# SaeedRahmani/AV-Simulation-at-Intersections

Measured on NVIDIA B200. Metric: batched MPC step solves/sec, higher is better.
Workload: dtype f64

## Files before the change

### av-simulation-at-intersections_b200/csrc/jmpc.cu

```cuda
#include <cuda_runtime.h>

#include <cstdio>
#include <cstdlib>
#include <cstring>
#include <new>
#include <string>
#include <chrono>
#include <vector>

#include "../../include/jmpc.h"
#include "jmpc_collision.cuh"
#include "jmpc_step.cuh"
#include "jmpc_episode.cuh"
#include "jmpc_planner.cuh"
#include "jmpc_courses.cuh"

namespace {

thread_local std::string g_err;

int fail(const char* what, cudaError_t e = cudaSuccess) {
  char buf[512];
  if (e != cudaSuccess) snprintf(buf, sizeof buf, "%s: %s", what, cudaGetErrorString(e));
  else snprintf(buf, sizeof buf, "%s", what);
// ... 1486 lines not shown
      B, h->n_courses, h->course_stride, course_id, course_ok, dl, h->d_cx, h->d_cy, h->d_cyaw, state, params, done);
  CK(cudaGetLastError());
  h->launches++;
  return 0;
}

int64_t jmpc_launch_count(jmpc_handle h) { return h ? h->launches : 0; }

int32_t jmpc_debug_linalg(jmpc_handle h, int32_t n, const double* A, const double* b, const double* x, double* sol,
                          double* prod) {
  return jmpc_debug_linalg_g(h, n, 32, 0, A, b, x, sol, prod);
}

int32_t jmpc_debug_linalg_g(jmpc_handle h, int32_t n, int32_t group_lanes, int32_t which, const double* A,
                            const double* b, const double* x, double* sol, double* prod) {
  if (!h || !A || !b || !x || !sol || !prod) return fail("jmpc_debug_linalg: NULL argument");
  if (n < 1 || n > 2 * JMPC_MAX_T) return fail("jmpc_debug_linalg: n out of range");
  if (group_lanes != 16 && group_lanes != 32) return fail("jmpc_debug_linalg: group_lanes must be 16 or 32");
  const int groups = 32 / group_lanes;
  if (which < 0 || which >= groups) return fail("jmpc_debug_linalg: no such lane group");
  CK(cudaSetDevice(h->device));
  const size_t nn = (size_t)n * n;
  const size_t in_doubles = nn + 2 * (size_t)n, out_doubles = 4 * (size_t)n + 2;
  if (ensure_stage(h, (in_doubles + out_doubles) * sizeof(double))) return -1;
  double* hs = (double*)h->h_stage;
  double* d = (double*)h->d_stage;
  memcpy(hs, A, nn * sizeof(double)); memcpy(hs + nn, b, n * sizeof(double)); memcpy(hs + nn + n, x, n * sizeof(double));
  double *dA = d, *db = dA + nn, *dx = db + n, *dsol = dx + n, *dprod = dsol + 2 * n;
  int* dok = (int*)(dprod + 2 * n);
  cudaStream_t st = h->own_stream;
  CK(cudaMemcpyAsync(d, hs, in_doubles * sizeof(double), cudaMemcpyHostToDevice, st));
  CK(cudaMemsetAsync(dsol, 0xff, out_doubles * sizeof(double), st));
  const int nb = jmpc::nblk(n);
  const size_t smem = (size_t)groups * (jmpc::tiles_doubles(n) + 8 * nb) * sizeof(double) +
                      jmpc::chol_lut_bytes(nb) + 16;
  if (group_lanes == 32) jmpc::linalg_selftest_kernel<32><<<1, 32, smem, st>>>(n, which, dA, db, dx, dsol, dprod, dok);
  else jmpc::linalg_selftest_kernel<16><<<1, 32, smem, st>>>(n, which, dA, db, dx, dsol, dprod, dok);
  CK(cudaGetLastError());
  h->launches++;
  CK(cudaMemcpyAsync(hs + in_doubles, dsol, out_doubles * sizeof(double), cudaMemcpyDeviceToHost, st));
  CK(cudaStreamSynchronize(st));
  memcpy(sol, hs + in_doubles, 2 * (size_t)n * sizeof(double));
  memcpy(prod, hs + in_doubles + 2 * n, 2 * (size_t)n * sizeof(double));
  int ok = 0;
  memcpy(&ok, hs + in_doubles + 4 * n, sizeof(int));
  return ok == 1 ? 0 : 1;
}

int32_t jmpc_measure_fma_peak(jmpc_handle h, double* fp64_tflops, double* fp32_tflops) {
  if (!h || !fp64_tflops || !fp32_tflops) return fail("jmpc_measure_fma_peak: NULL argument");
  CK(cudaSetDevice(h->device));
  if (measure_fma<double>(h, fp64_tflops)) return -1;
  if (measure_fma<float>(h, fp32_tflops)) return -1;
  return 0;
}

}
```

### av-simulation-at-intersections_b200/csrc/jmpc_linalg.cuh

```cuda
#pragma once
#include <cuda_runtime.h>
#include <math.h>

namespace jmpc {

#ifdef JMPC_UNROLL_BLOCKS
#define JMPC_PRAGMA_CHOL _Pragma("unroll")
#define JMPC_PRAGMA_SWEEP _Pragma("unroll")
#define JMPC_PRAGMA_SYMV _Pragma("unroll")
#else
#define JMPC_PRAGMA_CHOL _Pragma("unroll 1")
#define JMPC_PRAGMA_SWEEP _Pragma("unroll 1")
#define JMPC_PRAGMA_SYMV _Pragma("unroll 1")
#endif

#ifdef JMPC_CYCLES
__device__ unsigned long long g_cycles[32];
#define JMPC_TICK(var) long long var = clock64()
#define JMPC_TOCK(var, slot) do { long long now_ = clock64(); if ((threadIdx.x & 31) == 0) atomicAdd(&g_cycles[slot], (unsigned long long)(now_ - var)); var = now_; } while (0)
#else
#define JMPC_TICK(var)
#define JMPC_TOCK(var, slot)
#endif

constexpr int kTS = 18;
constexpr unsigned kFullMask = 0xffffffffu;

__host__ __device__ inline int nblk(int n) { return (n + 3) >> 2; }
__host__ __device__ inline int tiles_doubles(int n) { const int nb = nblk(n); return (nb * (nb + 1) / 2) * kTS; }
__host__ __device__ __forceinline__ int tile_off(int I, int J) { return (((I * (I + 1)) >> 1) + J) * kTS; }
__host__ __device__ __forceinline__ int elem_off(int i, int j) { return tile_off(i >> 2, j >> 2) + ((i & 3) << 2) + (j & 3); }

__device__ __forceinline__ double rsqrt_pos(double a) {
  double y;
  asm("rsqrt.approx.ftz.f64 %0, %1;" : "=d"(y) : "d"(a));
  const double e = fma(-a, y * y, 1.0);
  return fma(fma(e, 0.375, 0.5), y * e, y);
}
__device__ __forceinline__ double rcp_pos(double a) {
  double y;
  asm("rcp.approx.ftz.f64 %0, %1;" : "=d"(y) : "d"(a));
  double e = fma(-a, y, 1.0);
  y = fma(y, e, y);
  e = fma(-a, y, 1.0);
  return fma(y, e, y);
}
__device__ __forceinline__ double pivot_rsqrt(double a, bool& clean) {
  const double y = rsqrt_pos(a);
  const bool pos = a > 0.0;
  clean = clean && pos;
  return pos ? y : 0.0;
}

__device__ __forceinline__ void ld4(const double* p, double& a, double& b, double& c, double& d) {
  const double2 x = *reinterpret_cast<const double2*>(p), y = *reinterpret_cast<const double2*>(p + 2);
  a = x.x; b = x.y; c = y.x; d = y.y;
}
__device__ __forceinline__ void st4(double* p, double a, double b, double c, double d) {
  *reinterpret_cast<double2*>(p) = make_double2(a, b);
  *reinterpret_cast<double2*>(p + 2) = make_double2(c, d);
}

typedef unsigned int chol_task;
__host__ __device__ inline int chol_lut_entries(int nb) { return ((nb - 1) * nb * (nb + 1)) / 3; }
__host__ __device__ __forceinline__ int chol_lut_offset(int m) { return ((m - 1) * m * (m + 1)) / 3; }
__host__ __device__ inline size_t chol_lut_bytes(int nb) { return ((size_t)chol_lut_entries(nb) * sizeof(chol_task) + 15) & ~(size_t)15; }
__device__ inline void chol_lut_build(chol_task* lut, int nb, int tid, int nthreads) {
  for (int m = 1; m < nb; ++m) {
    const int ntasks = m * (m + 1), off = chol_lut_offset(m);
    const int J = nb - 1 - m;
    for (int q = tid; q < ntasks; q += nthreads) {
      const int t = q >> 1;
      int a = (int)((sqrtf(8.0f * (float)t + 1.0f) - 1.0f) * 0.5f);
      while (((a + 1) * (a + 2) >> 1) <= t) ++a;
      while (((a * (a + 1)) >> 1) > t) --a;
      const int b = t - ((a * (a + 1)) >> 1);
      const int I = J + 1 + a, Kc = J + 1 + b;
      lut[off + q] = ((unsigned)(b + 1) << 16) | ((unsigned)(q & 1) << 22) | (unsigned)(((I * (I + 1)) >> 1) + J) |
                     ((unsigned)(((Kc * (Kc + 1)) >> 1) + J) << 8);
    }
  }
}

template <int G>
__device__ inline bool chol_tiles(double* K, int nb, int gl, unsigned gm, const chol_task* lut,
                                  double* rhs = nullptr) {
  bool all_clean = true;
  JMPC_PRAGMA_CHOL
  for (int J = 0; J < nb; ++J) {
    JMPC_TICK(tc_);
    const double* D = K + tile_off(J, J);
    double a00, a10, a11, a20, a21, a22, a30, a31, a32, a33;
    {
      double u01, u02, u03, u12, u13, u23;
      ld4(D, a00, u01, u02, u03); ld4(D + 4, a10, a11, u12, u13);
      ld4(D + 8, a20, a21, a22, u23); ld4(D + 12, a30, a31, a32, a33);
      (void)u01; (void)u02; (void)u03; (void)u12; (void)u13; (void)u23;
    }
    bool clean = true;
    const double r0 = pivot_rsqrt(a00, clean);
    const double l10 = a10 * r0, l20 = a20 * r0, l30 = a30 * r0;
    a11 = fma(-l10, l10, a11);
    const double r1 = pivot_rsqrt(a11, clean);
    const double l21 = fma(-l20, l10, a21) * r1, l31 = fma(-l30, l10, a31) * r1;
    a22 = fma(-l21, l21, fma(-l20, l20, a22));
    const double r2 = pivot_rsqrt(a22, clean);
    const double l32 = fma(-l31, l21, fma(-l30, l20, a32)) * r2;
    a33 = fma(-l32, l32, fma(-l31, l31, fma(-l30, l30, a33)));
    const double r3 = pivot_rsqrt(a33, clean);
    all_clean = all_clean && clean;
    const double m00 = r0, m11 = r1, m22 = r2, m33 = r3;
    const double m10 = -(l10 * m00) * r1;
    const double m21 = -(l21 * m11) * r2;
    const double m32 = -(l32 * m22) * r3;
    const double m20 = -fma(l21, m10, l20 * m00) * r2;
    const double m31 = -fma(l32, m21, l31 * m11) * r3;
    const double m30 = -fma(l32, m20, fma(l31, m10, l30 * m00)) * r3;
    double y0 = 0.0, y1 = 0.0, y2 = 0.0, y3 = 0.0;
    if (rhs) {
      double b0, b1, b2, b3;
      ld4(rhs + (J << 2), b0, b1, b2, b3);
      y0 = m00 * b0; y1 = fma(m11, b1, m10 * b0); y2 = fma(m22, b2, fma(m21, b1, m20 * b0));
      y3 = fma(m31, b1, m30 * b0) + fma(m33, b3, m32 * b2);
    }
    __syncwarp(gm);
    JMPC_TOCK(tc_, 13);
    const int prow = (nb - J - 1) << 2;
    for (int r = gl; r < prow; r += G) {
      double* row = K + tile_off(J + 1 + (r >> 2), J) + ((r & 3) << 2);
      double a0, a1, a2, a3;
      ld4(row, a0, a1, a2, a3);
      const double x0 = a0 * m00, x1 = fma(a1, m11, a0 * m10), x2 = fma(a2, m22, fma(a1, m21, a0 * m20));
      const double x3 = fma(a3, m33, fma(a2, m32, fma(a1, m31, a0 * m30)));
      st4(row, x0, x1, x2, x3);
      if (rhs) {
        double* bi = rhs + ((J + 1) << 2) + r;
        *bi -= fma(x1, y1, x0 * y0) + fma(x3, y3, x2 * y2);
      }
    }
    if (gl == 0) {
      double* Mw = K + tile_off(J, J);
      st4(Mw, m00, 0.0, 0.0, 0.0); st4(Mw + 4, m10, m11, 0.0, 0.0);
      st4(Mw + 8, m20, m21, m22, 0.0); st4(Mw + 12, m30, m31, m32, m33);
      if (rhs) st4(rhs + (J << 2), y0, y1, y2, y3);
    }
    __syncwarp(gm);
    JMPC_TOCK(tc_, 14);
    const int m = nb - J - 1, ntasks = m * (m + 1);
    const chol_task* tasks = lut + chol_lut_offset(m);
    for (int q = gl; q < ntasks; q += G) {
      const unsigned e = tasks[q];
      const unsigned sLI = e & 255u, sLK = (e >> 8) & 255u, sC = sLI + ((e >> 16) & 15u), hb = (e >> 16) & 0x40u;
      const char* Kh = reinterpret_cast<const char*>(K) + hb;
      const double* LI = reinterpret_cast<const double*>(Kh + sLI * (unsigned)(kTS * sizeof(double)));
      const double* LK = K + sLK * (unsigned)kTS;
      double* C = reinterpret_cast<double*>(const_cast<char*>(Kh) + sC * (unsigned)(kTS * sizeof(double)));
      double k00, k01, k02, k03, k10, k11, k12, k13, k20, k21, k22, k23, k30, k31, k32, k33;
      ld4(LK, k00, k01, k02, k03); ld4(LK + 4, k10, k11, k12, k13);
      ld4(LK + 8, k20, k21, k22, k23); ld4(LK + 12, k30, k31, k32, k33);
#pragma unroll
      for (int r = 0; r < 2; ++r) {
        double x0, x1, x2, x3, c0, c1, c2, c3;
        ld4(LI + 4 * r, x0, x1, x2, x3);
        ld4(C + 4 * r, c0, c1, c2, c3);
        c0 = fma(-x3, k03, fma(-x2, k02, fma(-x1, k01, fma(-x0, k00, c0))));
        c1 = fma(-x3, k13, fma(-x2, k12, fma(-x1, k11, fma(-x0, k10, c1))));
        c2 = fma(-x3, k23, fma(-x2, k22, fma(-x1, k21, fma(-x0, k20, c2))));
        c3 = fma(-x3, k33, fma(-x2, k32, fma(-x1, k31, fma(-x0, k30, c3))));
        st4(C + 4 * r, c0, c1, c2, c3);
      }
    }
    __syncwarp(gm);
    JMPC_TOCK(tc_, 15);
  }
  return all_clean;
}

template <int G>
__device__ inline void solve_forward_tiles(const double* K, double* b, int nb, int gl, unsigned gm) {
  const int n4 = nb << 2;
  JMPC_PRAGMA_SWEEP
  for (int J = 0; J < nb; ++J) {
    const double* Mw = K + tile_off(J, J);
    double b0, b1, b2, b3;
    ld4(b + (J << 2), b0, b1, b2, b3);
    const double m00 = Mw[0];
    const double2 mr1 = *reinterpret_cast<const double2*>(Mw + 4);
    const double m10 = mr1.x, m11 = mr1.y;
    double m20, m21, m22, mpad, m30, m31, m32, m33;
    ld4(Mw + 8, m20, m21, m22, mpad); ld4(Mw + 12, m30, m31, m32, m33);
    (void)mpad;
    const double y0 = m00 * b0, y1 = fma(m11, b1, m10 * b0), y2 = fma(m22, b2, fma(m21, b1, m20 * b0));
    const double y3 = fma(m33, b3, fma(m32, b2, fma(m31, b1, m30 * b0)));
    __syncwarp(gm);
    for (int i = ((J + 1) << 2) + gl; i < n4; i += G) {
      double l0, l1, l2, l3;
      ld4(K + tile_off(i >> 2, J) + ((i & 3) << 2), l0, l1, l2, l3);
      b[i] = fma(-l3, y3, fma(-l2, y2, fma(-l1, y1, fma(-l0, y0, b[i]))));
    }
    if (gl == 0) st4(b + (J << 2), y0, y1, y2, y3);
    __syncwarp(gm);
  }
}
template <int G>
__device__ inline void solve_backward_tiles(const double* K, double* b, int nb, int gl, unsigned gm) {
  JMPC_PRAGMA_SWEEP
  for (int J = nb - 1; J >= 0; --J) {
    const double* Mw = K + tile_off(J, J);
    double y0, y1, y2, y3;
    ld4(b + (J << 2), y0, y1, y2, y3);
    const double m00 = Mw[0];
    const double2 mr1 = *reinterpret_cast<const double2*>(Mw + 4);
    const double m10 = mr1.x, m11 = mr1.y;
    double m20, m21, m22, mpad, m30, m31, m32, m33;
    ld4(Mw + 8, m20, m21, m22, mpad); ld4(Mw + 12, m30, m31, m32, m33);
    (void)mpad;
    const double x3 = m33 * y3, x2 = fma(m32, y3, m22 * y2), x1 = fma(m31, y3, fma(m21, y2, m11 * y1));
    const double x0 = fma(m30, y3, fma(m20, y2, fma(m10, y1, m00 * y0)));
    __syncwarp(gm);
    for (int i = gl; i < (J << 2); i += G) {
      const double* col = K + tile_off(J, i >> 2) + (i & 3);
      b[i] = fma(-col[12], x3, fma(-col[8], x2, fma(-col[4], x1, fma(-col[0], x0, b[i]))));
    }
    if (gl == 0) st4(b + (J << 2), x0, x1, x2, x3);
    __syncwarp(gm);
  }
}

template <int G>
__device__ __forceinline__ void sweep_load(const double* b, int n4, int gl, double& lo, double& hi) {
  lo = (gl < n4) ? b[gl] : 0.0;
  hi = (gl + G < n4) ? b[gl + G] : 0.0;
}
template <int G>
__device__ __forceinline__ void sweep_store(double* b, int n4, int gl, double lo, double hi) {
  if (gl < n4) b[gl] = lo;
  if (gl + G < n4) b[gl + G] = hi;
}
struct DiagInv { double m00, m10, m11, m20, m21, m22, m30, m31, m32, m33; };
__device__ __forceinline__ DiagInv load_diag_inv(const double* Mw) {
  DiagInv d;
  d.m00 = Mw[0];
  const double2 r1 = *reinterpret_cast<const double2*>(Mw + 4);
  d.m10 = r1.x; d.m11 = r1.y;
  double pad;
  ld4(Mw + 8, d.m20, d.m21, d.m22, pad); ld4(Mw + 12, d.m30, d.m31, d.m32, d.m33);
  (void)pad;
  return d;
}
template <int G, bool HI>
__device__ __forceinline__ void forward_block(const double* K, int J, int n4, int gl, unsigned gm, const double* row_lo,
                                              const double* row_hi, double& lo, double& hi) {
  double& own = HI ? hi : lo;
  const int l0 = (J << 2) & (G - 1);
  const double* Mw = K + tile_off(J, J);
  const int first = (J + 1) << 2;
  const bool act_lo = !HI && gl >= first && gl < n4, act_hi = gl + G >= first && gl + G < n4;
  double a0 = 0.0, a1 = 0.0, a2 = 0.0, a3 = 0.0, c0, c1, c2, c3;
  if (!HI) ld4(act_lo ? row_lo + J * kTS : Mw, a0, a1, a2, a3);
  ld4(act_hi ? row_hi + J * kTS : Mw, c0, c1, c2, c3);
  const DiagInv d = load_diag_inv(Mw);
  const double e0 = __shfl_sync(gm, own, l0, G), e1 = __shfl_sync(gm, own, l0 + 1, G);
  const double e2 = __shfl_sync(gm, own, l0 + 2, G), e3 = __shfl_sync(gm, own, l0 + 3, G);
  const double y0 = d.m00 * e0, y1 = fma(d.m11, e1, d.m10 * e0), y2 = fma(d.m22, e2, fma(d.m21, e1, d.m20 * e0));
  const double y3 = fma(d.m33, e3, fma(d.m32, e2, fma(d.m31, e1, d.m30 * e0)));
  if (!HI) {
    const double v = fma(-a3, y3, fma(-a2, y2, fma(-a1, y1, fma(-a0, y0, lo))));
    lo = act_lo ? v : lo;
  }
  {
    const double v = fma(-c3, y3, fma(-c2, y2, fma(-c1, y1, fma(-c0, y0, hi))));
    hi = act_hi ? v : hi;
  }
  const double s01 = (gl & 1) ? y1 : y0, s23 = (gl & 1) ? y3 : y2, mine = (gl & 2) ? s23 : s01;
  own = ((gl >> 2) == (l0 >> 2)) ? mine : own;
}
template <int G>
__device__ __forceinline__ void solve_forward_regs(const double* K, int nb, int gl, unsigned gm, double& lo, double& hi) {
  const int n4 = nb << 2;
  const double* row_lo = K + tile_off(gl >> 2, 0) + ((gl & 3) << 2);
  const double* row_hi = K + tile_off((gl + G) >> 2, 0) + ((gl & 3) << 2);
  const int nlo = nb < G / 4 ? nb : G / 4;
#pragma unroll 1
  for (int J = 0; J < nlo; ++J) forward_block<G, false>(K, J, n4, gl, gm, row_lo, row_hi, lo, hi);
#pragma unroll 1
  for (int J = G / 4; J < nb; ++J) forward_block<G, true>(K, J, n4, gl, gm, row_lo, row_hi, lo, hi);
}
template <int G, bool HI>
__device__ __forceinline__ void backward_block(const double* K, int J, int n4, int gl, unsigned gm, int col_lo, int col_hi,
                                               double& lo, double& hi) {
  double& own = HI ? hi : lo;
  const int l0 = (J << 2) & (G - 1);
  const double* Krow = K + tile_off(J, 0);
  const double* Mw = Krow + J * kTS;
  const int below = J << 2;
  const bool act_lo = gl < below && gl < n4, act_hi = HI && gl + G < below;
  const double* pa = act_lo ? Krow + col_lo : Mw;
  const double a0 = pa[0], a1 = pa[4], a2 = pa[8], a3 = pa[12];
  double c0 = 0.0, c1 = 0.0, c2 = 0.0, c3 = 0.0;
  if (HI) { const double* pc = act_hi ? Krow + col_hi : Mw; c0 = pc[0]; c1 = pc[4]; c2 = pc[8]; c3 = pc[12]; }
  const DiagInv d = load_diag_inv(Mw);
  const double y0 = __shfl_sync(gm, own, l0, G), y1 = __shfl_sync(gm, own, l0 + 1, G);
  const double y2 = __shfl_sync(gm, own, l0 + 2, G), y3 = __shfl_sync(gm, own, l0 + 3, G);
  const double x3 = d.m33 * y3, x2 = fma(d.m32, y3, d.m22 * y2), x1 = fma(d.m31, y3, fma(d.m21, y2, d.m11 * y1));
  const double x0 = fma(d.m30, y3, fma(d.m20, y2, fma(d.m10, y1, d.m00 * y0)));
  {
    const double v = fma(-a3, x3, fma(-a2, x2, fma(-a1, x1, fma(-a0, x0, lo))));
    lo = act_lo ? v : lo;
  }
  if (HI) {
    const double v = fma(-c3, x3, fma(-c2, x2, fma(-c1, x1, fma(-c0, x0, hi))));
    hi = act_hi ? v : hi;
  }
  const double s01 = (gl & 1) ? x1 : x0, s23 = (gl & 1) ? x3 : x2, mine = (gl & 2) ? s23 : s01;
  own = ((gl >> 2) == (l0 >> 2)) ? mine : own;
}
template <int G>
__device__ __forceinline__ void solve_backward_regs(const double* K, int nb, int gl, unsigned gm, double& lo, double& hi) {
  const int n4 = nb << 2;
  const int col_lo = (gl >> 2) * kTS + (gl & 3), col_hi = ((gl + G) >> 2) * kTS + (gl & 3);
#pragma unroll 1
  for (int J = nb - 1; J >= G / 4; --J) backward_block<G, true>(K, J, n4, gl, gm, col_lo, col_hi, lo, hi);
  const int nlo = nb < G / 4 ? nb : G / 4;
#pragma unroll 1
  for (int J = nlo - 1; J >= 0; --J) backward_block<G, false>(K, J, n4, gl, gm, col_lo, col_hi, lo, hi);
}

__device__ inline void symv_tiles(const double* P, const double* x, int nb, int lane,
                                  double& y0, double& y1) {
  const int n4 = nb << 2;
  y0 = 0.0; y1 = 0.0;
#pragma unroll
  for (int pass = 0; pass < 2; ++pass) {
    const int i = lane + 32 * pass;
    if (i < n4) {
      const int I = i >> 2, r = i & 3;
      double acc0 = 0.0, acc1 = 0.0;
      for (int J = 0; J <= I; ++J) {
        double p0, p1, p2, p3, x0, x1, x2, x3;
        ld4(P + tile_off(I, J) + (r << 2), p0, p1, p2, p3);
        ld4(x + (J << 2), x0, x1, x2, x3);
        acc0 = fma(p1, x1, fma(p0, x0, acc0));
        acc1 = fma(p3, x3, fma(p2, x2, acc1));
      }
      for (int J = I + 1; J < nb; ++J) {
        const double* col = P + tile_off(J, I) + r;
        double x0, x1, x2, x3;
        ld4(x + (J << 2), x0, x1, x2, x3);
        acc0 = fma(col[4], x1, fma(col[0], x0, acc0));
        acc1 = fma(col[12], x3, fma(col[8], x2, acc1));
      }
      if (pass == 0) y0 = acc0 + acc1; else y1 = acc0 + acc1;
    }
  }
}


template <int G>
__device__ inline void solve_tiles(const double* K, double* b, int nb, int gl, unsigned gm) {
  solve_forward_tiles<G>(K, b, nb, gl, gm);
  solve_backward_tiles<G>(K, b, nb, gl, gm);
}

template <int NB>
__device__ __forceinline__ void symv_rows(const double* P, const double* x, int T, int nb_rt, int gl, double& y0,
                                          double& y1) {
  const int nb = (NB > 0) ? NB : nb_rt;
  const bool own = gl < T;
  const int ia = own ? gl : 0, ib = own ? T + gl : 0;
  const int Ia = ia >> 2, Ib = ib >> 2;
  const double* rowa = P + tile_off(Ia, 0) + ((ia & 3) << 2);
  const double* rowb = P + tile_off(Ib, 0) + ((ib & 3) << 2);
  const double* cola = P + Ia * kTS + (ia & 3);
  const double* colb = P + Ib * kTS + (ib & 3);
  double a0 = 0.0, a1 = 0.0, a2 = 0.0, a3 = 0.0, b0 = 0.0, b1 = 0.0, b2 = 0.0, b3 = 0.0;
  JMPC_PRAGMA_SYMV
  for (int J = 0; J < nb; ++J) {
    double x0, x1, x2, x3, p0, p1, p2, p3;
    ld4(x + (J << 2), x0, x1, x2, x3);
    const int tj = ((J * (J + 1)) >> 1) * kTS;
    if (J <= Ia) ld4(rowa + J * kTS, p0, p1, p2, p3);
    else { const double* col = cola + tj; p0 = col[0]; p1 = col[4]; p2 = col[8]; p3 = col[12]; }
    a0 = fma(p0, x0, a0); a1 = fma(p1, x1, a1); a2 = fma(p2, x2, a2); a3 = fma(p3, x3, a3);
    if (J <= Ib) ld4(rowb + J * kTS, p0, p1, p2, p3);
    else { const double* col = colb + tj; p0 = col[0]; p1 = col[4]; p2 = col[8]; p3 = col[12]; }
    b0 = fma(p0, x0, b0); b1 = fma(p1, x1, b1); b2 = fma(p2, x2, b2); b3 = fma(p3, x3, b3);
  }
  y0 = own ? (a0 + a1) + (a2 + a3) : 0.0;
  y1 = own ? (b0 + b1) + (b2 + b3) : 0.0;
}

template <int G>
__global__ void linalg_selftest_kernel(int n, int which, const double* __restrict__ A, const double* __restrict__ b,
                                       const double* __restrict__ x, double* __restrict__ sol,
                                       double* __restrict__ prod, int* __restrict__ ok) {
  extern __shared__ double sm[];
  const int lane = threadIdx.x & 31, gl = lane & (G - 1), sub = lane / G, nb = nblk(n), n4 = nb << 2;
  const unsigned gm = (G == 32) ? kFullMask : (((1u << (G & 31)) - 1u) << (sub * G));
  const int per_group = tiles_doubles(n) + 2 * n4;
  double* K = sm + sub * per_group;
  double* rhs = K + tiles_doubles(n);
  double* xv = rhs + n4;
  chol_task* lut = reinterpret_cast<chol_task*>(sm + (32 / G) * per_group);
  chol_lut_build(lut, nb, lane, 32);
  __syncwarp();
  const bool report = sub == which;
  auto pack = [&]() {
    for (int e = gl; e < tiles_doubles(n); e += G) K[e] = 0.0;
    __syncwarp(gm);
    for (int e = gl; e < n4 * n4; e += G) {
      const int i = e / n4, j = e % n4;
      if (j > i && (i >> 2) != (j >> 2)) continue;
      K[elem_off(i, j)] = (i < n && j < n) ? A[i * n + j] : ((i == j) ? 1.0 : 0.0);
    }
    __syncwarp(gm);
  };
  pack();
  for (int i = gl; i < n4; i += G) { rhs[i] = (i < n) ? b[i] : 0.0; xv[i] = (i < n) ? x[i] : 0.0; }
  __syncwarp(gm);
  if (G == 32) {
    double y0, y1;
    symv_tiles(K, xv, nb, lane, y0, y1);
    if (lane < n) prod[lane] = y0;
    if (lane + 32 < n) prod[lane + 32] = y1;
    __syncwarp(gm);
  }
  const bool good = chol_tiles<G>(K, nb, gl, gm, lut);
  {
    double lo, hi, lo2, hi2;
    sweep_load<G>(rhs, n4, gl, lo2, hi2);
    solve_tiles<G>(K, rhs, nb, gl, gm);
    __syncwarp(gm);
    sweep_load<G>(rhs, n4, gl, lo, hi);
    solve_forward_regs<G>(K, nb, gl, gm, lo2, hi2);
    solve_backward_regs<G>(K, nb, gl, gm, lo2, hi2);
    const bool same = (lo == lo2 || (lo != lo && lo2 != lo2)) && (hi == hi2 || (hi != hi && hi2 != hi2));
    __syncwarp(gm);
    sweep_store<G>(rhs, n4, gl, same ? lo : nan(""), same ? hi : nan(""));
  }
  __syncwarp(gm);
  if (report) {
    for (int i = gl; i < n; i += G) sol[i] = rhs[i];
    if (gl == 0) *ok = good ? 1 : 0;
  }
  if ((n & 1) == 0 && (n >> 1) <= G) {
    const int T = n >> 1;
    __syncwarp(gm);
    pack();
    double q0, q1;
    symv_rows<0>(K, xv, T, nb, gl, q0, q1);
    if (report && gl < T) { prod[n + gl] = q0; prod[n + T + gl] = q1; }
  }
}

}
```

### av-simulation-at-intersections_b200/csrc/jmpc_step.cuh

```cuda
#pragma once
#include <cuda_runtime.h>
#include <stdint.h>
#include <math.h>

#include "../../include/jmpc.h"
#include "jmpc_linalg.cuh"

namespace jmpc {

constexpr int kMaxT = JMPC_MAX_T;
constexpr unsigned kFull = 0xffffffffu;

struct ParamVec { double v[JMPC_NPARAM]; };

struct StepArgs {
  int B, T;
  int lin_iters;
  int max_iters;
  double mu_tol;
  double tol_res;
  double init_mu;
  double du_th;
  const double* cx; const double* cy; const double* cyaw;
  const double* cv;
// ... 12 lines not shown
  int n_peers;
  long long rank_offset;
  unsigned long long* peer_flag[JMPC_MAX_PEERS];
  int n_flag_peers;
  unsigned long long gather_step;
  unsigned int* blocks_done;
  double* pscratch;
  unsigned int* counter;
};

constexpr int kSlotHi3 = JMPC_NPARAM, kSlotLo3 = JMPC_NPARAM + 1, kSlotLim = JMPC_NPARAM + 2;
constexpr int kSlotGscale = JMPC_NPARAM + 3;
constexpr int kParamSlots = 32;
static_assert(JMPC_NPARAM + 4 <= kParamSlots, "parameter block too small");

enum MomentSlot {
  MOM_11, MOM_11_B, MOM_11_BB,
  MOM_12, MOM_12_B, MOM_12_K, MOM_12_BK,
  MOM_22, MOM_22_K, MOM_22_KK,
  MOM_QPSI, MOM_WX, MOM_WY, MOM_COUNT
};

__host__ __device__ inline int even_up(int x) { return (x + 1) & ~1; }
__host__ __device__ inline int k_region_doubles(int T) {
  const int a = tiles_doubles(2 * T), b = MOM_COUNT * even_up(T + 1);
  return a > b ? a : b;
}
#ifndef JMPC_PAD_T1E
#define JMPC_PAD_T1E 0
#endif
__host__ __device__ inline int inst_smem_doubles(int T) {
  const int n = 2 * T, n4 = nblk(n) << 2, T1e = even_up(T + 1), Te = even_up(T);
  return k_region_doubles(T)
         + 4 * n4
         + (9 + JMPC_PAD_T1E) * T1e
         + 4 * Te
         + kParamSlots
         + 2;
}

__host__ __device__ inline int group_lanes_for(int T) { return (T + 1 <= 16) ? 16 : 32; }

__host__ __device__ inline size_t step_block_smem_bytes(int T, int wpb, int groups) {
  return (size_t)wpb * groups * inst_smem_doubles(T) * sizeof(double) + chol_lut_bytes(nblk(2 * T));
}

__device__ __forceinline__ int tri(int i) { return (i * (i + 1)) >> 1; }

template <int G>
__device__ __forceinline__ unsigned group_mask(int lane) {
  if constexpr (G == 32) return kFull;
  else return ((1u << G) - 1u) << (lane & ~(G - 1));
}
__device__ __forceinline__ double dmax(double a, double b) { return a > b ? a : b; }
template <int G>
__device__ __forceinline__ double grp_sum(double v, unsigned gm) {
#pragma unroll
  for (int o = G / 2; o > 0; o >>= 1) v += __shfl_xor_sync(gm, v, o);
  return v;
}
template <int G>
__device__ __forceinline__ double grp_max(double v, unsigned gm) {
#pragma unroll
  for (int o = G / 2; o > 0; o >>= 1) v = dmax(v, __shfl_xor_sync(gm, v, o));
  return v;
}
template <int G>
// ... 78 lines not shown
                                    int start, double x, double y, int gl, unsigned gm) {
  const int m = n_course - start;
  if (m <= 1) return start;
  if (m == 2) return start + 1;
  Near3 s;
  s.d0 = s.d1 = s.d2 = INFINITY;
  s.i0 = s.i1 = s.i2 = 0x7fffffff;
  for (int j = start + gl; j < n_course; j += G) {
    const double ex = cx[j] - x, ey = cy[j] - y;
    const double d = __dadd_rn(__dmul_rn(ex, ex), __dmul_rn(ey, ey));
    near3_insert(s, d, j - start);
  }
  int res[3];
#pragma unroll
  for (int r = 0; r < 3; ++r) {
    double bd = s.d0; int bi = s.i0;
#pragma unroll
    for (int o = G / 2; o > 0; o >>= 1) {
      const double od = __shfl_xor_sync(gm, bd, o);
      const int oi = __shfl_xor_sync(gm, bi, o);
      if (closer(od, oi, bd, bi)) { bd = od; bi = oi; }
    }
    res[r] = bi;
    if (s.i0 == bi) {
      s.d0 = s.d1; s.i0 = s.i1; s.d1 = s.d2; s.i1 = s.i2; s.d2 = INFINITY; s.i2 = 0x7fffffff;
    }
  }
  if (abs(res[1] - res[2]) == 2) return res[0] + start;
  if (abs(res[0] - res[1]) == 1) return max(res[0], res[1]) + start;
  return -1;
}

struct WarpMem {
  double *K, *u, *q, *rhs, *grad;
  double *alp, *cb, *wvs, *ck;
  double *WeX, *WeY, *epsi, *vb, *th;
  double *wA, *wD, *wR, *wS;
  double *prm;
  unsigned long long* mbar;
  __device__ WarpMem(double* base, int T) {
    const int n = 2 * T, n4 = nblk(n) << 2, T1e = even_up(T + 1), Te = even_up(T);
    double* p = base;
    K = p; p += k_region_doubles(T);
    u = p; p += n4; q = p; p += n4; rhs = p; p += n4; grad = p; p += n4;
    alp = p; p += T1e; cb = p; p += T1e; wvs = p; p += T1e; ck = p; p += T1e;
    WeX = p; p += T1e; WeY = p; p += T1e; epsi = p; p += T1e;
    p += JMPC_PAD_T1E * T1e;
    vb = p; p += T1e; th = p; p += T1e;
    wA = p; p += Te; wD = p; p += Te; wR = p; p += Te; wS = p; p += Te;
    prm = p; p += kParamSlots;
    mbar = reinterpret_cast<unsigned long long*>(p);
  }
};

__device__ __forceinline__ unsigned smem_u32(const void* p) { return (unsigned)__cvta_generic_to_shared(p); }
__device__ __forceinline__ void mbar_init(unsigned long long* bar, unsigned count) {
  asm volatile("mbarrier.init.shared::cta.b64 [%0], %1;\n" ::"r"(smem_u32(bar)), "r"(count) : "memory");
  asm volatile("fence.mbarrier_init.release.cluster;\n" ::: "memory");
}
__device__ __forceinline__ void tma_load_1d(void* smem_dst, const void* gmem_src, unsigned bytes, unsigned long long* bar) {
  asm volatile("fence.proxy.async;\n" ::: "memory");
  asm volatile("mbarrier.arrive.expect_tx.shared::cta.b64 _, [%0], %1;\n" ::"r"(smem_u32(bar)), "r"(bytes) : "memory");
  asm volatile("cp.async.bulk.shared::cluster.global.mbarrier::complete_tx::bytes [%0], [%1], %2, [%3];\n"
               ::"r"(smem_u32(smem_dst)), "l"(gmem_src), "r"(bytes), "r"(smem_u32(bar)) : "memory");
}
__device__ __forceinline__ void mbar_wait(unsigned long long* bar, unsigned parity) {
  unsigned done;
  do {
    asm volatile("{\n .reg .pred p;\n mbarrier.try_wait.parity.shared::cta.b64 p, [%1], %2;\n selp.u32 %0, 1, 0, p;\n}\n"
                 : "=r"(done) : "r"(smem_u32(bar)), "r"(parity) : "memory");
  } while (!done);
}

template <int G>
__device__ __forceinline__ void rows_apply(const double* u, int T, int gl, unsigned gm, double z[4]) {
  const double sk = (gl < T) ? u[gl] : 0.0, sm = (gl >= 1 && gl <= T) ? u[gl - 1] : 0.0;
  const double d = (gl < T) ? u[T + gl] : 0.0;
  const double dn = __shfl_down_sync(gm, d, 1, G);
  z[0] = sk - sm; z[1] = d; z[2] = dn - d; z[3] = sk;
}
template <int G>
__device__ __forceinline__ void rows_apply_reg(double a, double d, int gl, unsigned gm, bool live013, bool live2,
// ... 359 lines not shown
    rows_apply_T<G>(t4, gl, gm, ra, rd);
    const double g0 = (gl < T) ? pu0 + M.q[gl] + ra : 0.0, g1 = (gl < T) ? pu1 + M.q[T + gl] + rd : 0.0;
    __syncwarp(gm);
    JMPC_TOCK(ts_, 2);
    if (gl < T) {
      const int i = T + gl;
      M.K[elem_off(gl, gl)] += M.wA[gl];
      M.K[elem_off(i, i)] += M.wD[gl];
      if (gl >= 1) { M.K[elem_off(gl, gl - 1)] -= M.wS[gl]; M.K[elem_off(i, i - 1)] -= M.wR[gl - 1]; }
    }
    const double rdmax_l = dmax(fabs(g0), fabs(g1));
    const bool rp_strict = grp_all<G>(rpmax <= A.tol_res), rp_red = grp_all<G>(rpmax <= 1e-7), rp_brk = grp_all<G>(rpmax <= 1e-9);
    const double gscale = M.prm[kSlotGscale];
    const bool rd_strict = grp_all<G>(rdmax_l <= A.tol_res * gscale), rd_red = grp_all<G>(rdmax_l <= 1e-7 * gscale);
    const bool rd_brk = grp_all<G>(rdmax_l <= 1e-9 * gscale);
#ifdef JMPC_DEBUG_RESID
    const double rpmax_g = grp_max<G>(rpmax, gm), rdmax = grp_max<G>(rdmax_l, gm);
#endif
    __syncwarp(gm);
    if (!kLock || !done) {
      if (mu <= A.mu_tol && rp_strict && rd_strict) { converged = true; done = true; }
      else if (mu <= 1e-3 * A.mu_tol && rp_strict) { converged = true; done = true; }
      else acceptable = (mu <= 1e-9 && rp_red && rd_red);
      if (kLock && done) my_iters = it;
#ifdef JMPC_DEBUG_RESID
      dbg_mu = mu; dbg_rp = rpmax_g; dbg_rd = rdmax / gscale;
#endif
    }
    if (kLock ? __all_sync(kFull, done) : done) break;

    JMPC_TOCK(ts_, 3);
    if (gl < T) { M.rhs[gl] = -g0 - ra_p; M.rhs[T + gl] = -g1 - rd_p; }
    __syncwarp(gm);
    const bool clean = chol_tiles<G>(M.K, nb, gl, gm, lut, M.rhs);
    JMPC_TOCK(ts_, 4);
    if ((!kLock || !done) && !clean && mu <= 1e-11 && rp_brk && rd_brk) {
      acceptable = true; done = true;
      if (kLock) my_iters = it;
    }
    if (!kLock && done) break;

    double dsh[4], dsl[4], dlh[4], dll[4];
    double aff_step = 0.0;
#pragma unroll 1
    for (int phase = 0; phase < 2; ++phase) {
      double sw_lo = 0.0, sw_hi = 0.0;
      (void)sw_lo; (void)sw_hi;
      auto rp = [&](int k) -> double { return (gl < T) ? stash[k * T + gl] : 0.0; };
      if (phase == 1) {
        double th[4], ish[4], isl[4];
        slack_rcp(sh, sl, ish, isl);
#pragma unroll
        for (int r = 0; r < 4; ++r) {
          const double a_l = __dmul_rn(fma(ll[r], rp(4 + r), -dll[r]), isl[r]);
          th[r] = fma(fma(lh[r], rp(r), -dlh[r]), ish[r], -a_l);
        }
        rows_apply_T<G>(th, gl, gm, ra, rd);
        if (gl < T) { M.rhs[gl] = -g0 - ra; M.rhs[T + gl] = -g1 - rd; }
        __syncwarp(gm);
        JMPC_TOCK(ts_, 5);
        if constexpr (LAT) {
          sweep_load<G>(M.rhs, nb << 2, gl, sw_lo, sw_hi);
          solve_forward_regs<G>(M.K, nb, gl, gm, sw_lo, sw_hi);
        } else {
          solve_forward_tiles<G>(M.K, M.rhs, nb, gl, gm);
        }
      } else {
        if constexpr (LAT) sweep_load<G>(M.rhs, nb << 2, gl, sw_lo, sw_hi);
#pragma unroll
        for (int r = 0; r < 4; ++r) { dlh[r] = lh[r] * sh[r]; dll[r] = ll[r] * sl[r]; }
        JMPC_TOCK(ts_, 5);
      }
      if constexpr (LAT) {
        solve_backward_regs<G>(M.K, nb, gl, gm, sw_lo, sw_hi);
        __syncwarp(gm);
        sweep_store<G>(M.rhs, nb << 2, gl, sw_lo, sw_hi);
      } else {
        solve_backward_tiles<G>(M.K, M.rhs, nb, gl, gm);
      }
      __syncwarp(gm);
      if (phase == 1 && gl == 0 && it + 1 < A.max_iters) tma_load_1d(M.K, pscr, (unsigned)(ntd * sizeof(double)), M.mbar);
      const double du0 = (gl < T) ? M.rhs[gl] : 0.0, du1 = (gl < T) ? M.rhs[T + gl] : 0.0;
      JMPC_TOCK(ts_, 6);
      double dz[4];
      rows_apply_reg<G>(du0, du1, gl, gm, live013, live2, dz);
      double rho = 0.0, wn = 0.0, wd = 1.0, ish[4], isl[4];
      slack_rcp(sh, sl, ish, isl);
      auto cand = [&](double num, double den) { if (num * wd > wn * den) { wn = num; wd = den; } };
#pragma unroll
      for (int r = 0; r < 4; ++r) {
        const double rch = dlh[r], rcl = dll[r];
        dsh[r] = -rp(r) - dz[r];
        dsl[r] = -rp(4 + r) + dz[r];
        dlh[r] = -(fma(lh[r], dsh[r], rch)) * ish[r];
        dll[r] = -(fma(ll[r], dsl[r], rcl)) * isl[r];
        rho = dmax(rho, dmax(-dsh[r] * ish[r], -dsl[r] * isl[r]));
        cand(-dlh[r], lh[r]); cand(-dll[r], ll[r]);
      }
      rho = dmax(rho, wn * rcp_pos(wd));
      rho = grp_max<G>(rho, gm);
      const double amax = (rho > 0.5) ? rcp_pos(rho) : 2.0;
      if (phase == 0) {
        const double aa = fmin(1.0, amax);
        aff_step = aa;
        double mu_aff = 0.0;
#pragma unroll
        for (int r = 0; r < 4; ++r)
          mu_aff += fma(aa, dlh[r], lh[r]) * fma(aa, dsh[r], sh[r]) + fma(aa, dll[r], ll[r]) * fma(aa, dsl[r], sl[r]);
        mu_aff = grp_sum<G>(mu_aff, gm) * inv_rows;
        const double ratio = mu_aff * rcp_pos(mu);
        const double sigma_mu = ratio * ratio * ratio * mu;
// ... 300 lines not shown
```

Before: 5.979 million.

## Store Cholesky diagonal inverses in separate buffer and split forward/back solve buffers

The inverted 4x4 diagonal blocks now go into a compact per-warp dinv array instead of being written back over the diagonal tiles of K. Forward and backward solves write into a separate y buffer, so results are no longer stored in place over the rhs. This lets one __syncwarp per block step in the factorization and both tile solves be dropped, which shortens the serial critical path. In exchange the solver uses more shared memory per instance, which could lower occupancy, and the dinv pointer is aliased into the grad region, which risks overlapping other data.

```diff
diff --git a/av-simulation-at-intersections_b200/csrc/jmpc.cu b/av-simulation-at-intersections_b200/csrc/jmpc.cu
--- a/av-simulation-at-intersections_b200/csrc/jmpc.cu
+++ b/av-simulation-at-intersections_b200/csrc/jmpc.cu
@@ -1542,10 +1542,15 @@
   CK(cudaMemcpyAsync(d, hs, in_doubles * sizeof(double), cudaMemcpyHostToDevice, st));
   CK(cudaMemsetAsync(dsol, 0xff, out_doubles * sizeof(double), st));
   const int nb = jmpc::nblk(n);
-  const size_t smem = (size_t)groups * (jmpc::tiles_doubles(n) + 8 * nb) * sizeof(double) +
+  const size_t smem = (size_t)groups * jmpc::selftest_group_doubles(n) * sizeof(double) +
                       jmpc::chol_lut_bytes(nb) + 16;
-  if (group_lanes == 32) jmpc::linalg_selftest_kernel<32><<<1, 32, smem, st>>>(n, which, dA, db, dx, dsol, dprod, dok);
-  else jmpc::linalg_selftest_kernel<16><<<1, 32, smem, st>>>(n, which, dA, db, dx, dsol, dprod, dok);
+  if (group_lanes == 32) {
+    CK(cudaFuncSetAttribute(jmpc::linalg_selftest_kernel<32>, cudaFuncAttributeMaxDynamicSharedMemorySize, (int)smem));
+    jmpc::linalg_selftest_kernel<32><<<1, 32, smem, st>>>(n, which, dA, db, dx, dsol, dprod, dok);
+  } else {
+    CK(cudaFuncSetAttribute(jmpc::linalg_selftest_kernel<16>, cudaFuncAttributeMaxDynamicSharedMemorySize, (int)smem));
+    jmpc::linalg_selftest_kernel<16><<<1, 32, smem, st>>>(n, which, dA, db, dx, dsol, dprod, dok);
+  }
   CK(cudaGetLastError());
   h->launches++;
   CK(cudaMemcpyAsync(hs + in_doubles, dsol, out_doubles * sizeof(double), cudaMemcpyDeviceToHost, st));
diff --git a/av-simulation-at-intersections_b200/csrc/jmpc_linalg.cuh b/av-simulation-at-intersections_b200/csrc/jmpc_linalg.cuh
--- a/av-simulation-at-intersections_b200/csrc/jmpc_linalg.cuh
+++ b/av-simulation-at-intersections_b200/csrc/jmpc_linalg.cuh
@@ -15,9 +15,12 @@
 #endif
 
 #ifdef JMPC_CYCLES
+#ifndef JMPC_CYCLES_EVERY
+#define JMPC_CYCLES_EVERY 1
+#endif
 __device__ unsigned long long g_cycles[32];
 #define JMPC_TICK(var) long long var = clock64()
-#define JMPC_TOCK(var, slot) do { long long now_ = clock64(); if ((threadIdx.x & 31) == 0) atomicAdd(&g_cycles[slot], (unsigned long long)(now_ - var)); var = now_; } while (0)
+#define JMPC_TOCK(var, slot) do { long long now_ = clock64(); if ((threadIdx.x & 31) == 0 && ((blockIdx.x * blockDim.x + threadIdx.x) >> 5) % JMPC_CYCLES_EVERY == 0) atomicAdd(&g_cycles[slot], (unsigned long long)(now_ - var)); var = now_; } while (0)
 #else
 #define JMPC_TICK(var)
 #define JMPC_TOCK(var, slot)
@@ -82,9 +85,22 @@
   }
 }
 
-template <int G>
-__device__ inline bool chol_tiles(double* K, int nb, int gl, unsigned gm, const chol_task* lut,
-                                  double* rhs = nullptr) {
+constexpr int kDI = 10;
+__host__ __device__ inline int diag_inv_doubles(int nb) { return kDI * nb; }
+struct DiagInv { double m00, m10, m11, m20, m21, m22, m30, m31, m32, m33; };
+__device__ __forceinline__ DiagInv load_diag_inv(const double* p) {
+  DiagInv d;
+  const double2 a = reinterpret_cast<const double2*>(p)[0], b = reinterpret_cast<const double2*>(p)[1];
+  const double2 c = reinterpret_cast<const double2*>(p)[2], e = reinterpret_cast<const double2*>(p)[3];
+  const double2 f = reinterpret_cast<const double2*>(p)[4];
+  d.m00 = a.x; d.m10 = a.y; d.m11 = b.x; d.m20 = b.y; d.m21 = c.x; d.m22 = c.y;
+  d.m30 = e.x; d.m31 = e.y; d.m32 = f.x; d.m33 = f.y;
+  return d;
+}
+
+template <int G>
+__device__ inline bool chol_tiles(double* K, double* dinv, int nb, int gl, unsigned gm, const chol_task* lut,
+                                  double* rhs = nullptr, double* y = nullptr) {
   bool all_clean = true;
   JMPC_PRAGMA_CHOL
   for (int J = 0; J < nb; ++J) {
@@ -123,7 +139,12 @@
       y0 = m00 * b0; y1 = fma(m11, b1, m10 * b0); y2 = fma(m22, b2, fma(m21, b1, m20 * b0));
       y3 = fma(m31, b1, m30 * b0) + fma(m33, b3, m32 * b2);
     }
-    __syncwarp(gm);
+    if (gl == 0) {
+      double2* Mw = reinterpret_cast<double2*>(dinv + kDI * J);
+      Mw[0] = make_double2(m00, m10); Mw[1] = make_double2(m11, m20); Mw[2] = make_double2(m21, m22);
+      Mw[3] = make_double2(m30, m31); Mw[4] = make_double2(m32, m33);
+      if (rhs) st4(y + (J << 2), y0, y1, y2, y3);
+    }
     JMPC_TOCK(tc_, 13);
     const int prow = (nb - J - 1) << 2;
     for (int r = gl; r < prow; r += G) {
@@ -137,12 +158,6 @@
         double* bi = rhs + ((J + 1) << 2) + r;
         *bi -= fma(x1, y1, x0 * y0) + fma(x3, y3, x2 * y2);
       }
-    }
-    if (gl == 0) {
-      double* Mw = K + tile_off(J, J);
-      st4(Mw, m00, 0.0, 0.0, 0.0); st4(Mw + 4, m10, m11, 0.0, 0.0);
-      st4(Mw + 8, m20, m21, m22, 0.0); st4(Mw + 12, m30, m31, m32, m33);
-      if (rhs) st4(rhs + (J << 2), y0, y1, y2, y3);
     }
     __syncwarp(gm);
     JMPC_TOCK(tc_, 14);
@@ -177,52 +192,40 @@
 }
 
 template <int G>
-__device__ inline void solve_forward_tiles(const double* K, double* b, int nb, int gl, unsigned gm) {
+__device__ inline void solve_forward_tiles(const double* K, const double* dinv, double* b, double* y, int nb, int gl,
+                                           unsigned gm) {
   const int n4 = nb << 2;
   JMPC_PRAGMA_SWEEP
   for (int J = 0; J < nb; ++J) {
-    const double* Mw = K + tile_off(J, J);
     double b0, b1, b2, b3;
     ld4(b + (J << 2), b0, b1, b2, b3);
-    const double m00 = Mw[0];
-    const double2 mr1 = *reinterpret_cast<const double2*>(Mw + 4);
-    const double m10 = mr1.x, m11 = mr1.y;
-    double m20, m21, m22, mpad, m30, m31, m32, m33;
-    ld4(Mw + 8, m20, m21, m22, mpad); ld4(Mw + 12, m30, m31, m32, m33);
-    (void)mpad;
-    const double y0 = m00 * b0, y1 = fma(m11, b1, m10 * b0), y2 = fma(m22, b2, fma(m21, b1, m20 * b0));
-    const double y3 = fma(m33, b3, fma(m32, b2, fma(m31, b1, m30 * b0)));
-    __syncwarp(gm);
+    const DiagInv d = load_diag_inv(dinv + kDI * J);
+    const double y0 = d.m00 * b0, y1 = fma(d.m11, b1, d.m10 * b0), y2 = fma(d.m22, b2, fma(d.m21, b1, d.m20 * b0));
+    const double y3 = fma(d.m33, b3, fma(d.m32, b2, fma(d.m31, b1, d.m30 * b0)));
     for (int i = ((J + 1) << 2) + gl; i < n4; i += G) {
       double l0, l1, l2, l3;
       ld4(K + tile_off(i >> 2, J) + ((i & 3) << 2), l0, l1, l2, l3);
       b[i] = fma(-l3, y3, fma(-l2, y2, fma(-l1, y1, fma(-l0, y0, b[i]))));
     }
-    if (gl == 0) st4(b + (J << 2), y0, y1, y2, y3);
-    __syncwarp(gm);
-  }
-}
-template <int G>
-__device__ inline void solve_backward_tiles(const double* K, double* b, int nb, int gl, unsigned gm) {
+    if (gl == 0) st4(y + (J << 2), y0, y1, y2, y3);
+    __syncwarp(gm);
+  }
+}
+template <int G>
+__device__ inline void solve_backward_tiles(const double* K, const double* dinv, double* y, double* x, int nb, int gl,
+                                            unsigned gm) {
   JMPC_PRAGMA_SWEEP
   for (int J = nb - 1; J >= 0; --J) {
-    const double* Mw = K + tile_off(J, J);
     double y0, y1, y2, y3;
-    ld4(b + (J << 2), y0, y1, y2, y3);
-    const double m00 = Mw[0];
-    const double2 mr1 = *reinterpret_cast<const double2*>(Mw + 4);
-    const double m10 = mr1.x, m11 = mr1.y;
-    double m20, m21, m22, mpad, m30, m31, m32, m33;
-    ld4(Mw + 8, m20, m21, m22, mpad); ld4(Mw + 12, m30, m31, m32, m33);
-    (void)mpad;
-    const double x3 = m33 * y3, x2 = fma(m32, y3, m22 * y2), x1 = fma(m31, y3, fma(m21, y2, m11 * y1));
-    const double x0 = fma(m30, y3, fma(m20, y2, fma(m10, y1, m00 * y0)));
-    __syncwarp(gm);
+    ld4(y + (J << 2), y0, y1, y2, y3);
+    const DiagInv d = load_diag_inv(dinv + kDI * J);
+    const double x3 = d.m33 * y3, x2 = fma(d.m32, y3, d.m22 * y2), x1 = fma(d.m31, y3, fma(d.m21, y2, d.m11 * y1));
+    const double x0 = fma(d.m30, y3, fma(d.m20, y2, fma(d.m10, y1, d.m00 * y0)));
     for (int i = gl; i < (J << 2); i += G) {
       const double* col = K + tile_off(J, i >> 2) + (i & 3);
-      b[i] = fma(-col[12], x3, fma(-col[8], x2, fma(-col[4], x1, fma(-col[0], x0, b[i]))));
-    }
-    if (gl == 0) st4(b + (J << 2), x0, x1, x2, x3);
+      y[i] = fma(-col[12], x3, fma(-col[8], x2, fma(-col[4], x1, fma(-col[0], x0, y[i]))));
+    }
+    if (gl == 0) st4(x + (J << 2), x0, x1, x2, x3);
     __syncwarp(gm);
   }
 }
@@ -237,20 +240,9 @@
   if (gl < n4) b[gl] = lo;
   if (gl + G < n4) b[gl + G] = hi;
 }
-struct DiagInv { double m00, m10, m11, m20, m21, m22, m30, m31, m32, m33; };
-__device__ __forceinline__ DiagInv load_diag_inv(const double* Mw) {
-  DiagInv d;
-  d.m00 = Mw[0];
-  const double2 r1 = *reinterpret_cast<const double2*>(Mw + 4);
-  d.m10 = r1.x; d.m11 = r1.y;
-  double pad;
-  ld4(Mw + 8, d.m20, d.m21, d.m22, pad); ld4(Mw + 12, d.m30, d.m31, d.m32, d.m33);
-  (void)pad;
-  return d;
-}
 template <int G, bool HI>
-__device__ __forceinline__ void forward_block(const double* K, int J, int n4, int gl, unsigned gm, const double* row_lo,
-                                              const double* row_hi, double& lo, double& hi) {
+__device__ __forceinline__ void forward_block(const double* K, const double* dinv, int J, int n4, int gl, unsigned gm,
+                                              const double* row_lo, const double* row_hi, double& lo, double& hi) {
   double& own = HI ? hi : lo;
   const int l0 = (J << 2) & (G - 1);
   const double* Mw = K + tile_off(J, J);
@@ -259,7 +251,7 @@
   double a0 = 0.0, a1 = 0.0, a2 = 0.0, a3 = 0.0, c0, c1, c2, c3;
   if (!HI) ld4(act_lo ? row_lo + J * kTS : Mw, a0, a1, a2, a3);
   ld4(act_hi ? row_hi + J * kTS : Mw, c0, c1, c2, c3);
-  const DiagInv d = load_diag_inv(Mw);
+  const DiagInv d = load_diag_inv(dinv + kDI * J);
   const double e0 = __shfl_sync(gm, own, l0, G), e1 = __shfl_sync(gm, own, l0 + 1, G);
   const double e2 = __shfl_sync(gm, own, l0 + 2, G), e3 = __shfl_sync(gm, own, l0 + 3, G);
   const double y0 = d.m00 * e0, y1 = fma(d.m11, e1, d.m10 * e0), y2 = fma(d.m22, e2, fma(d.m21, e1, d.m20 * e0));
@@ -276,19 +268,20 @@
   own = ((gl >> 2) == (l0 >> 2)) ? mine : own;
 }
 template <int G>
-__device__ __forceinline__ void solve_forward_regs(const double* K, int nb, int gl, unsigned gm, double& lo, double& hi) {
+__device__ __forceinline__ void solve_forward_regs(const double* K, const double* dinv, int nb, int gl, unsigned gm,
+                                                   double& lo, double& hi) {
   const int n4 = nb << 2;
   const double* row_lo = K + tile_off(gl >> 2, 0) + ((gl & 3) << 2);
   const double* row_hi = K + tile_off((gl + G) >> 2, 0) + ((gl & 3) << 2);
   const int nlo = nb < G / 4 ? nb : G / 4;
 #pragma unroll 1
-  for (int J = 0; J < nlo; ++J) forward_block<G, false>(K, J, n4, gl, gm, row_lo, row_hi, lo, hi);
+  for (int J = 0; J < nlo; ++J) forward_block<G, false>(K, dinv, J, n4, gl, gm, row_lo, row_hi, lo, hi);
 #pragma unroll 1
-  for (int J = G / 4; J < nb; ++J) forward_block<G, true>(K, J, n4, gl, gm, row_lo, row_hi, lo, hi);
+  for (int J = G / 4; J < nb; ++J) forward_block<G, true>(K, dinv, J, n4, gl, gm, row_lo, row_hi, lo, hi);
 }
 template <int G, bool HI>
-__device__ __forceinline__ void backward_block(const double* K, int J, int n4, int gl, unsigned gm, int col_lo, int col_hi,
-                                               double& lo, double& hi) {
+__device__ __forceinline__ void backward_block(const double* K, const double* dinv, int J, int n4, int gl, unsigned gm,
+                                               int col_lo, int col_hi, double& lo, double& hi) {
   double& own = HI ? hi : lo;
   const int l0 = (J << 2) & (G - 1);
   const double* Krow = K + tile_off(J, 0);
@@ -299,7 +292,7 @@
   const double a0 = pa[0], a1 = pa[4], a2 = pa[8], a3 = pa[12];
   double c0 = 0.0, c1 = 0.0, c2 = 0.0, c3 = 0.0;
   if (HI) { const double* pc = act_hi ? Krow + col_hi : Mw; c0 = pc[0]; c1 = pc[4]; c2 = pc[8]; c3 = pc[12]; }
-  const DiagInv d = load_diag_inv(Mw);
+  const DiagInv d = load_diag_inv(dinv + kDI * J);
   const double y0 = __shfl_sync(gm, own, l0, G), y1 = __shfl_sync(gm, own, l0 + 1, G);
   const double y2 = __shfl_sync(gm, own, l0 + 2, G), y3 = __shfl_sync(gm, own, l0 + 3, G);
   const double x3 = d.m33 * y3, x2 = fma(d.m32, y3, d.m22 * y2), x1 = fma(d.m31, y3, fma(d.m21, y2, d.m11 * y1));
@@ -316,14 +309,15 @@
   own = ((gl >> 2) == (l0 >> 2)) ? mine : own;
 }
 template <int G>
-__device__ __forceinline__ void solve_backward_regs(const double* K, int nb, int gl, unsigned gm, double& lo, double& hi) {
+__device__ __forceinline__ void solve_backward_regs(const double* K, const double* dinv, int nb, int gl, unsigned gm,
+                                                    double& lo, double& hi) {
   const int n4 = nb << 2;
   const int col_lo = (gl >> 2) * kTS + (gl & 3), col_hi = ((gl + G) >> 2) * kTS + (gl & 3);
 #pragma unroll 1
-  for (int J = nb - 1; J >= G / 4; --J) backward_block<G, true>(K, J, n4, gl, gm, col_lo, col_hi, lo, hi);
+  for (int J = nb - 1; J >= G / 4; --J) backward_block<G, true>(K, dinv, J, n4, gl, gm, col_lo, col_hi, lo, hi);
   const int nlo = nb < G / 4 ? nb : G / 4;
 #pragma unroll 1
-  for (int J = nlo - 1; J >= 0; --J) backward_block<G, false>(K, J, n4, gl, gm, col_lo, col_hi, lo, hi);
+  for (int J = nlo - 1; J >= 0; --J) backward_block<G, false>(K, dinv, J, n4, gl, gm, col_lo, col_hi, lo, hi);
 }
 
 __device__ inline void symv_tiles(const double* P, const double* x, int nb, int lane,
@@ -357,9 +351,10 @@
 
 
 template <int G>
-__device__ inline void solve_tiles(const double* K, double* b, int nb, int gl, unsigned gm) {
-  solve_forward_tiles<G>(K, b, nb, gl, gm);
-  solve_backward_tiles<G>(K, b, nb, gl, gm);
+__device__ inline void solve_tiles(const double* K, const double* dinv, double* b, double* tmp, int nb, int gl,
+                                   unsigned gm) {
+  solve_forward_tiles<G>(K, dinv, b, tmp, nb, gl, gm);
+  solve_backward_tiles<G>(K, dinv, tmp, b, nb, gl, gm);
 }
 
 template <int NB>
@@ -390,6 +385,7 @@
   y1 = own ? (b0 + b1) + (b2 + b3) : 0.0;
 }
 
+__host__ __device__ inline int selftest_group_doubles(int n) { return tiles_doubles(n) + 12 * nblk(n) + diag_inv_doubles(nblk(n)); }
 template <int G>
 __global__ void linalg_selftest_kernel(int n, int which, const double* __restrict__ A, const double* __restrict__ b,
                                        const double* __restrict__ x, double* __restrict__ sol,
@@ -397,10 +393,12 @@
   extern __shared__ double sm[];
   const int lane = threadIdx.x & 31, gl = lane & (G - 1), sub = lane / G, nb = nblk(n), n4 = nb << 2;
   const unsigned gm = (G == 32) ? kFullMask : (((1u << (G & 31)) - 1u) << (sub * G));
-  const int per_group = tiles_doubles(n) + 2 * n4;
+  const int per_group = selftest_group_doubles(n);
   double* K = sm + sub * per_group;
   double* rhs = K + tiles_doubles(n);
   double* xv = rhs + n4;
+  double* tmp = xv + n4;
+  double* dinv = tmp + n4;
   chol_task* lut = reinterpret_cast<chol_task*>(sm + (32 / G) * per_group);
   chol_lut_build(lut, nb, lane, 32);
   __syncwarp();
@@ -425,15 +423,15 @@
     if (lane + 32 < n) prod[lane + 32] = y1;
     __syncwarp(gm);
   }
-  const bool good = chol_tiles<G>(K, nb, gl, gm, lut);
+  const bool good = chol_tiles<G>(K, dinv, nb, gl, gm, lut);
   {
     double lo, hi, lo2, hi2;
     sweep_load<G>(rhs, n4, gl, lo2, hi2);
-    solve_tiles<G>(K, rhs, nb, gl, gm);
+    solve_tiles<G>(K, dinv, rhs, tmp, nb, gl, gm);
     __syncwarp(gm);
     sweep_load<G>(rhs, n4, gl, lo, hi);
-    solve_forward_regs<G>(K, nb, gl, gm, lo2, hi2);
-    solve_backward_regs<G>(K, nb, gl, gm, lo2, hi2);
+    solve_forward_regs<G>(K, dinv, nb, gl, gm, lo2, hi2);
+    solve_backward_regs<G>(K, dinv, nb, gl, gm, lo2, hi2);
     const bool same = (lo == lo2 || (lo != lo && lo2 != lo2)) && (hi == hi2 || (hi != hi && hi2 != hi2));
     __syncwarp(gm);
     sweep_store<G>(rhs, n4, gl, same ? lo : nan(""), same ? hi : nan(""));
diff --git a/av-simulation-at-intersections_b200/csrc/jmpc_step.cuh b/av-simulation-at-intersections_b200/csrc/jmpc_step.cuh
--- a/av-simulation-at-intersections_b200/csrc/jmpc_step.cuh
+++ b/av-simulation-at-intersections_b200/csrc/jmpc_step.cuh
@@ -68,7 +68,7 @@
 __host__ __device__ inline int inst_smem_doubles(int T) {
   const int n = 2 * T, n4 = nblk(n) << 2, T1e = even_up(T + 1), Te = even_up(T);
   return k_region_doubles(T)
-         + 4 * n4
+         + 5 * n4
          + (9 + JMPC_PAD_T1E) * T1e
          + 4 * Te
          + kParamSlots
@@ -213,22 +213,24 @@
 }
 
 struct WarpMem {
-  double *K, *u, *q, *rhs, *grad;
+  double *K, *u, *q, *rhs, *y, *grad;
   double *alp, *cb, *wvs, *ck;
   double *WeX, *WeY, *epsi, *vb, *th;
   double *wA, *wD, *wR, *wS;
+  double *dinv;
   double *prm;
   unsigned long long* mbar;
   __device__ WarpMem(double* base, int T) {
     const int n = 2 * T, n4 = nblk(n) << 2, T1e = even_up(T + 1), Te = even_up(T);
     double* p = base;
     K = p; p += k_region_doubles(T);
-    u = p; p += n4; q = p; p += n4; rhs = p; p += n4; grad = p; p += n4;
+    u = p; p += n4; q = p; p += n4; rhs = p; p += n4; y = p; p += n4; grad = p; p += n4;
     alp = p; p += T1e; cb = p; p += T1e; wvs = p; p += T1e; ck = p; p += T1e;
     WeX = p; p += T1e; WeY = p; p += T1e; epsi = p; p += T1e;
+    wA = p; p += Te; wD = p; p += Te; wR = p; p += Te; wS = p; p += Te;
+    dinv = grad + 8 * T;
     p += JMPC_PAD_T1E * T1e;
     vb = p; p += T1e; th = p; p += T1e;
-    wA = p; p += Te; wD = p; p += Te; wR = p; p += Te; wS = p; p += Te;
     prm = p; p += kParamSlots;
     mbar = reinterpret_cast<unsigned long long*>(p);
   }
@@ -654,7 +656,7 @@
     JMPC_TOCK(ts_, 3);
     if (gl < T) { M.rhs[gl] = -g0 - ra_p; M.rhs[T + gl] = -g1 - rd_p; }
     __syncwarp(gm);
-    const bool clean = chol_tiles<G>(M.K, nb, gl, gm, lut, M.rhs);
+    const bool clean = chol_tiles<G>(M.K, M.dinv, nb, gl, gm, lut, M.rhs, M.y);
     JMPC_TOCK(ts_, 4);
     if ((!kLock || !done) && !clean && mu <= 1e-11 && rp_brk && rd_brk) {
       acceptable = true; done = true;
@@ -683,22 +685,22 @@
         JMPC_TOCK(ts_, 5);
         if constexpr (LAT) {
           sweep_load<G>(M.rhs, nb << 2, gl, sw_lo, sw_hi);
-          solve_forward_regs<G>(M.K, nb, gl, gm, sw_lo, sw_hi);
+          solve_forward_regs<G>(M.K, M.dinv, nb, gl, gm, sw_lo, sw_hi);
         } else {
-          solve_forward_tiles<G>(M.K, M.rhs, nb, gl, gm);
+          solve_forward_tiles<G>(M.K, M.dinv, M.rhs, M.y, nb, gl, gm);
         }
       } else {
-        if constexpr (LAT) sweep_load<G>(M.rhs, nb << 2, gl, sw_lo, sw_hi);
+        if constexpr (LAT) sweep_load<G>(M.y, nb << 2, gl, sw_lo, sw_hi);
 #pragma unroll
         for (int r = 0; r < 4; ++r) { dlh[r] = lh[r] * sh[r]; dll[r] = ll[r] * sl[r]; }
         JMPC_TOCK(ts_, 5);
       }
       if constexpr (LAT) {
-        solve_backward_regs<G>(M.K, nb, gl, gm, sw_lo, sw_hi);
+        solve_backward_regs<G>(M.K, M.dinv, nb, gl, gm, sw_lo, sw_hi);
         __syncwarp(gm);
         sweep_store<G>(M.rhs, nb << 2, gl, sw_lo, sw_hi);
       } else {
-        solve_backward_tiles<G>(M.K, M.rhs, nb, gl, gm);
+        solve_backward_tiles<G>(M.K, M.dinv, M.y, M.rhs, nb, gl, gm);
       }
       __syncwarp(gm);
       if (phase == 1 && gl == 0 && it + 1 < A.max_iters) tma_load_1d(M.K, pscr, (unsigned)(ntd * sizeof(double)), M.mbar);
```

Result: faster. 6.082 million, median of 6 (+1.7%).
